# sarath-srinivas/PyGPR

Hardware: AMD Instinct MI355X
Metric: NLML+grad evals/sec at N=16384 D=8 RBF (higher is better)
Workload: dtype f64; 1 GPU; BASELINE config 3: one exact-GP NLML+gradient evaluation per GPU per step, N=16384 D=8, Compose([Squared_exponential, White_noise]), hp sigma=1 l=1 sigma_n=0.1, jitter 1e-7; N>1: grBCM shared-hp co-training (each rank's expert = 1024 global + 15360 own points), one all-reduce of [1+nhp] per step; experts_per_gpu=1

## Files before the change

pygpr_amd/_lib.py:

```python
import ctypes as C
import os
import re

_HERE = os.path.dirname(os.path.abspath(__file__))
LIB_PATH = os.path.join(_HERE, "lib", "libpygpr_hip.so")
HEADER = os.path.join(os.path.dirname(_HERE), "include", "pygpr_hip.h")
HEADER_LOO = os.path.join(os.path.dirname(_HERE), "include", "pygpr_hip_loo.h")
HEADER_SAMPLE = os.path.join(os.path.dirname(_HERE), "include", "pygpr_hip_sample.h")
HEADER_SPARSE = os.path.join(os.path.dirname(_HERE), "include", "pygpr_hip_sparse.h")
HEADER_SELECT = os.path.join(os.path.dirname(_HERE), "include", "pygpr_hip_select.h")
HEADER_MATMUL = os.path.join(os.path.dirname(_HERE), "include", "pygpr_hip_matmul.h")
HEADER_LOWRANK = os.path.join(os.path.dirname(_HERE), "include", "pygpr_hip_lowrank.h")
HEADER_FEATURE = os.path.join(os.path.dirname(_HERE), "include", "pygpr_hip_feature.h")
HEADER_DMATMUL = os.path.join(os.path.dirname(_HERE), "include", "pygpr_hip_dmatmul.h")
HEADER_ROWSQ = os.path.join(os.path.dirname(_HERE), "include", "pygpr_hip_rowsq.h")
HEADER_LXGRAD = os.path.join(os.path.dirname(_HERE), "include", "pygpr_hip_lxgrad.h")

PG_F64, PG_F32 = 0, 1
PG_KIND_RBF, PG_KIND_MATERN52, PG_KIND_SQDIST, PG_KIND_MATERN32, PG_KIND_MATERN12 = 0, 1, 2, 3, 4
PG_KIND_RQ = 6
PG_KIND_PERIODIC = 8
PG_MAX_COMP, PG_MAX_DIM = 4, 64
PG_SPEC_PRODUCT = int(re.search(r"#define\s+PG_SPEC_PRODUCT\s+(0[xX][0-9a-fA-F]+|\d+)", open(HEADER).read()).group(1), 0)
PAD = 256

GEMM_NT, GEMM_NT_RP, GEMM_NN, GEMM_TN, GEMM_TT, GEMM_NT_64, GEMM_NT_64x128, GEMM_NT_32x64, GEMM_NT_32x128, GEMM_TT_64, GEMM_NT_32x32 = 0, 1, 2, 3, 5, 6, 7, 8, 9, 10, 11
GEMM_TN_64 = 13


class CovSpec(C.Structure):
    _fields_ = [
        ("ncomp", C.c_int),
        ("kind", C.c_int * PG_MAX_COMP),
        ("off", C.c_int * PG_MAX_COMP),
        ("nnoise", C.c_int),
        ("noise_off", C.c_int * PG_MAX_COMP),
    ]


_RESTYPES = {"int": C.c_int, "long": C.c_long, "const char*": C.c_char_p}
_ARGTYPES = {"int": C.c_int, "long": C.c_long, "double": C.c_double, "const pg_covspec*": C.POINTER(CovSpec)}
_ARGTYPES.update((t, C.c_void_p) for t in ("pg_handle", "pg_handle*", "void*", "const void*", "double*", "const double*", "int*", "long*"))


def _strip_comments(text):
    return re.sub(r"/\*.*?\*/", "", text, flags=re.S)


def header_symbols():
    return sorted(set(re.findall(r"\b(pg_[a-z_0-9]+)\s*\(", _strip_comments(open(HEADER).read()))))


def parse_prototypes(text):
    def norm(t):
        return re.sub(r"\s*\*", "*", " ".join(t.split()))

    protos = {}
    for ret, name, params in re.findall(r"([\w \t*]+?)\b(pg_[a-z_0-9]+)\s*\(([^()]*)\)\s*;", _strip_comments(text)):
        types = []
        for p in [q.strip() for q in params.split(",")] if params.strip() != "void" else []:
            m = re.fullmatch(r"(.*[\s*])[A-Za-z_]\w*", p, flags=re.S)
            if not m:
                raise ValueError("%s: cannot read parameter %r" % (name, p))
            types.append(norm(m.group(1)))
        protos[name] = (norm(ret), types)
    return protos


def signatures(protos):
    sigs = {}
    for name, (ret, params) in protos.items():
        for t, table in [(ret, _RESTYPES)] + [(p, _ARGTYPES) for p in params]:
            if t not in table:
                raise ValueError("%s: no ctypes mapping for the type %r" % (name, t))
        sigs[name] = (_RESTYPES[ret], [_ARGTYPES[p] for p in params])
    return sigs


_SIGS = signatures(parse_prototypes(open(HEADER).read()))
_SIGS_LOO = signatures(parse_prototypes(open(HEADER_LOO).read()))
# ... 58 lines not shown
```

pygpr_amd/csrc/capi.hip:

```cpp
#include "gemm.h"
#include "kbuild.h"
#include "leaf.h"
#include "chainstep.h"
#include "linalg.h"
#include "pygpr_hip_loo.h"
#include "pygpr_hip_sample.h"
#include "sparse.h"
#include "select.h"
#include "kmatmul.h"
#include "dmatmul.h"
#include "krowsq.h"
#include "fmatmul.h"
#include "lowrank.h"
#include "lxgrad.h"
#include <cstdarg>
#include <cstdint>
#include <cstdio>
#include <cstdlib>
#include <cstring>
#include <mutex>
#include <vector>

static thread_local char g_err[512] = "";

// ... 54 lines not shown
    if (h && h->tmo_host) {
        const int v = *(volatile int*)h->tmo_host;
        if (v) {
            *(volatile int*)h->tmo_host = 0;
            if (h->coupled) {
                h->tmo_off = 1; h->calls_since_tmo = 0;
                if (h->rearms > h->rearms_seen) { h->rearm_cur = std::min(4096, std::max(1, h->rearm_cur) * 2); h->rearms_seen = h->rearms; }
            }
            h->coupled = 0;
            if (v != h->counted_epoch) {
                h->counted_epoch = v;
                h->timeouts += 1;
            }
        }
    }
}

static int join_side(pg_ctx* h, void* stream) {
    poll_timeout(h);
    if (h && h->side_pending) {
        PG_CHECK(hipStreamWaitEvent(ST(stream), h->ev[5], 0));
        if (ST(stream) == h->side_owner) h->side_pending = 0;
    }
    return 0;
}
#define JOIN(h, stream)                         \
    do {                                        \
        int _j = join_side((h), (stream));      \
        if (_j) return _j;                      \
    } while (0)

static int plain_device_memory(const void* p) {
    hipPointerAttribute_t a;
    if (hipPointerGetAttributes(&a, p) != hipSuccess) {
        (void)hipGetLastError();
        return 0;
    }
    return a.type == hipMemoryTypeDevice && !a.isManaged && !(a.allocationFlags & hipDeviceMallocFinegrained);
}
struct AtomicGuard {
    pg_ctx* h;
    AtomicGuard(pg_ctx* h_, const void* c) : h(h_) { if (h) h->no_atomic_c = plain_device_memory(c) ? 0 : 1; }
    ~AtomicGuard() { if (h) h->no_atomic_c = 0; }
};

template <typename T>
static int gemm_raw_t(pg_handle h, int variant, int M, int N, int K, double alpha, const void* A, long lda, const void* B,
                      long ldb, double beta, void* C, long ldc, int tri, int klo, int khi, void* stream) {
    GemmP<T> p;
    p.A = (const T*)A; p.B = (const T*)B; p.C = (T*)C;
    p.lda = lda; p.ldb = ldb; p.ldc = ldc;
    p.M = M; p.N = N; p.K = K;
    p.alpha = (T)alpha; p.beta = (T)beta;
    p.tri = tri; p.klo = klo & 3; p.khi = khi; p.krev = (klo >> 2) & 1;
    p.sA = p.sB = p.sC = 0; p.batch = 1;
    p.nexp = 1; p.eA = p.eB = p.eC = 0; p.einfo = 0;
    p.part = nullptr; p.ldp = 0; p.info = nullptr; p.noxcd = 0;
    static const char* rs = getenv("PG_RAW_STREAM");
    hipStream_t on = ST(stream);
    if (rs && rs[0] == 'u' && h->upd) on = h->upd;
    if (on == ST(stream)) return pg_gemm<T>(h, on, variant, p);
    PG_CHECK(hipEventRecord(h->ev[2], ST(stream)));
    PG_CHECK(hipStreamWaitEvent(on, h->ev[2], 0));
    const int rc = pg_gemm<T>(h, on, variant, p);
    PG_CHECK(hipEventRecord(h->ev[3], on));
    PG_CHECK(hipStreamWaitEvent(ST(stream), h->ev[3], 0));
    return rc;
}

__global__ void pg_probe_wait_kernel(int* flag, int* seen) {
    int ok = 0;
    for (int it = 0; it < 4096 && !ok; ++it) {
        ok = __hip_atomic_load(flag, __ATOMIC_RELAXED, __HIP_MEMORY_SCOPE_SYSTEM) != 0;
        __builtin_amdgcn_s_sleep(32);
    }
    __hip_atomic_store(seen, ok ? 1 : 2, __ATOMIC_RELAXED, __HIP_MEMORY_SCOPE_SYSTEM);
}
__global__ void pg_probe_set_kernel(int* flag) { __hip_atomic_store(flag, 1, __ATOMIC_RELAXED, __HIP_MEMORY_SCOPE_SYSTEM); }

static int probe_concurrent_queues(pg_ctx* c) {
    if (!c->probe_words && hipHostMalloc(reinterpret_cast<void**>(&c->probe_words), 64, hipHostMallocMapped) != hipSuccess) {
        (void)hipGetLastError();
        c->probe_words = nullptr;
        return 0;
    }
    int* words = c->probe_words;
    words[0] = 0;
    words[1] = 0;
    int* dwords = nullptr;
    int ok = 0;
    if (hipHostGetDevicePointer(reinterpret_cast<void**>(&dwords), words, 0) == hipSuccess) {
        hipLaunchKernelGGL(pg_probe_wait_kernel, dim3(1), dim3(1), 0, c->aux, dwords, dwords + 1);
        hipLaunchKernelGGL(pg_probe_set_kernel, dim3(1), dim3(1), 0, c->rows, dwords);
        if (hipStreamSynchronize(c->aux) == hipSuccess && hipStreamSynchronize(c->rows) == hipSuccess) ok = words[1] == 1;
    }
    (void)hipGetLastError();
    return ok;
}

static void maybe_rearm(pg_ctx* h) {
    if (h && h->coupled && h->rearms > 0 && h->rearm_cur > h->rearm_after && ++h->calls_since_rearm > h->rearm_cur) {
        h->rearm_cur = h->rearm_after;
        h->calls_since_rearm = 0;
    }
    if (!h || !h->tmo_off || h->coupled || h->rearm_after <= 0) return;
    if (h->rearm_cur < h->rearm_after) h->rearm_cur = h->rearm_after;
    if (++h->calls_since_tmo <= h->rearm_cur) return;
    h->calls_since_tmo = 0;
    if (h->rows && h->spin_ticks >= 0 && probe_concurrent_queues(h)) {
        h->coupled = 1;
// ... 980 lines not shown
    int* w = reinterpret_cast<int*>(scratch);
    const CsWait cw = {w + 1, nullptr, pg_wait_ticks(h, n), 1};
    return pg_spin_probe_launch(ST(stream), w, cw, reinterpret_cast<long long*>(w + 4));
}
int pg_chain_timeouts(pg_handle h) {
    if (!h) return -1;
    poll_timeout(h);
    return h->timeouts;
}

int pg_build_potrf_trtri_checked(pg_handle h, int dtype, const pg_covspec* spec, const double* hp, const void* X, long ldx, int n,
                                 int d, double jitter, void* A, long lda, int n_pad, void* inv_diag, int* info, void* Minv, long ldm,
                                 void* stream, int* info_host) {
    NEED(info_host, "null pointer");
    for (int attempt = 0; attempt < 2; ++attempt) {
        const int rc = pg_build_potrf_trtri(h, dtype, spec, hp, X, ldx, n, d, jitter, A, lda, n_pad, inv_diag, info, Minv, ldm, stream);
        if (rc) return rc;
        PG_CHECK(hipMemcpyAsync(info_host, info, sizeof(int), hipMemcpyDeviceToHost, ST(stream)));
        PG_CHECK(hipStreamSynchronize(ST(stream)));
        if (*info_host >= 0) return 0;
        poll_timeout(h);
        if (h->coupled) { h->tmo_off = 1; h->calls_since_tmo = 0; }
        h->coupled = 0;
    }
    return 0;
}

int pg_leaf_raw(pg_handle h, int dtype, void* A, long lda, void* inv, long ldi, int* info, void* stream) {
    JOIN(h, stream);
    NEED(h && A && info, "null pointer");
    return dispatch(dtype, __func__, [&](auto t) { using T = decltype(t);
        return pg_leaf<T>(ST(stream), (T*)A, lda, (T*)inv, ldi, info, 0);
    });
}

int pg_rowstep_raw(pg_handle h, int dtype, int n, void* A, long lda, int o0, int k0, const void* inv, int* flags, int* info, void* stream) {
    JOIN(h, stream);
    NEED(h && A && inv && flags && info, "null pointer");
    NEED(n % 128 == 0 && k0 % 128 == 0 && o0 % 128 == 0 && o0 <= k0 && k0 + 128 < n, "bad shape");
    PG_CHECK(hipMemsetAsync(flags, 0x40, 8 * sizeof(int), ST(stream)));
    PG_CHECK(hipMemsetAsync(flags + 6, 0, 2 * sizeof(int), ST(stream)));
    const CsWait cw = {flags + 6, nullptr, 200000000LL, 1};
    return dispatch(dtype, __func__, [&](auto t) { using T = decltype(t);
        return pg_rowstep<T>(ST(stream), (T*)A, lda, n, o0, k0, 1, (const T*)inv, flags, flags + 1, flags + 2, cw, info, flags + 3, flags + 4, 0);
    });
}

int pg_gemm_raw(pg_handle h, int dtype, int variant, int M, int N, int K, double alpha, const void* A, long lda,
                const void* B, long ldb, double beta, void* C, long ldc, int tri, int klo, int khi, void* stream) {
    JOIN(h, stream);
    NEED(h && A && B && C, "null pointer");
    NEED(variant == GEMM_NT_128 || variant == GEMM_NT_RP || variant == GEMM_NN_128 || variant == GEMM_TN_128 ||
             variant == GEMM_TT_128 || variant == GEMM_NT_64 || variant == GEMM_NT_64x128 || variant == GEMM_NT_32x64 ||
             variant == GEMM_NT_32x128 || variant == GEMM_TT_64 || variant == GEMM_NT_32x32 || variant == GEMM_TN_64,
         "variant not exposed");
    NEED16(A, lda); NEED16(B, ldb); NEED16(C, ldc);
    AtomicGuard ag(h, C);
    return dispatch(dtype, __func__, [&](auto t) {
        return gemm_raw_t<decltype(t)>(h, variant, M, N, K, alpha, A, lda, B, ldb, beta, C, ldc, tri, klo, khi, stream);
    });
}

}
```

pygpr_amd/csrc/gemm.h:

```cpp
#pragma once
#include "common.h"

template <typename T> struct GemmP {
    const T* A;
    const T* B;
    T* C;
    long lda, ldb, ldc;
    int M, N, K;
    T alpha, beta;
    int tri;
    int klo, khi;
    int krev;
    long sA, sB, sC;
    int batch;
    int nexp;
    long eA, eB, eC;
    int einfo;
    T* part;
    long ldp;
    const int* info;
    int noxcd;
    int atomic_c;
};

enum GemmVariant {
    GEMM_NT_128 = 0,
    GEMM_NT_RP = 1,
    GEMM_NN_128 = 2,
    GEMM_TN_128 = 3,
    GEMM_NN_128_SS = 4,
    GEMM_TT_128 = 5,
    GEMM_NT_64 = 6,
    GEMM_NT_64x128 = 7,
    GEMM_NT_32x64 = 8,
    GEMM_NT_32x128 = 9,
    GEMM_TT_64 = 10,
    GEMM_NT_128_SS = 12,
    GEMM_TN_64 = 13,
    GEMM_NT_32x32 = 11
};

template <typename T> int pg_gemm(pg_ctx* ctx, hipStream_t st, int variant, const GemmP<T>& p);
double pg_gemm_flops(int variant, int M, int N, int K, int tri, int klo, int khi, int batch);
```

pygpr_amd/csrc/gemm.hip:

```cpp
#include "gemm.h"
#include <cstdlib>
#include <cstdio>

#define BK 16

template <typename T, int R, bool KCONT, int BKT = BK, int NTH = 256> struct Stage {
    static constexpr int VE = 16 / sizeof(T);
    static constexpr int NV = (R * BKT / VE) / NTH;
    static_assert(NV >= 1, "fewer 16-byte vectors in the stage than threads");
    static constexpr int LDS_ELEMS = KCONT ? R * (BKT + 2) : BKT * (R + 16);
    typedef T vec_t __attribute__((ext_vector_type(VE)));
    typedef T half_t __attribute__((ext_vector_type(VE / 2)));
    vec_t v[NV];
    unsigned boff[NV];

    __device__ __forceinline__ void init(long ld, int tid) {
#pragma unroll
        for (int q = 0; q < NV; ++q) {
            const int idx = tid + NTH * q;
            if (KCONT) {
                const int row = idx / (BKT / VE), kv = idx % (BKT / VE);
                boff[q] = (unsigned)(((long)row * ld + kv * VE) * (long)sizeof(T));
            } else {
                const int kr = idx / (R / VE), rv = idx % (R / VE);
                boff[q] = (unsigned)(((long)kr * ld + rv * VE) * (long)sizeof(T));
            }
        }
    }
    static __device__ __forceinline__ const T* origin(const T* __restrict__ g, long ld, int r0, int k0) {
        return KCONT ? g + (long)r0 * ld + k0 : g + (long)k0 * ld + r0;
    }
    __device__ __forceinline__ void load(const T* __restrict__ org) {
        const char* b = reinterpret_cast<const char*>(org);
#pragma unroll
        for (int q = 0; q < NV; ++q) v[q] = *reinterpret_cast<const vec_t*>(b + (size_t)boff[q]);
    }
    __device__ __forceinline__ void store(T* s, int tid) const {
#pragma unroll
        for (int q = 0; q < NV; ++q) {
            const int idx = tid + NTH * q;
            if (KCONT) {
                const int row = idx / (BKT / VE), kv = idx % (BKT / VE);
                T* d = s + row * (BKT + 2) + kv * VE;
                half_t lo, hi;
#pragma unroll
                for (int e = 0; e < VE / 2; ++e) { lo[e] = v[q][e]; hi[e] = v[q][e + VE / 2]; }
                if (sizeof(T) == 8) {
                    *reinterpret_cast<vec_t*>(d) = v[q];
                } else {
                    *reinterpret_cast<half_t*>(d) = lo;
                    *reinterpret_cast<half_t*>(d + VE / 2) = hi;
                }
            } else {
                const int kr = idx / (R / VE), rv = idx % (R / VE);
                *reinterpret_cast<vec_t*>(s + kr * (R + 16) + rv * VE) = v[q];
            }
        }
    }
    static __device__ __forceinline__ T frag(const T* s, int r, int k) {
        return KCONT ? s[r * (BKT + 2) + k] : s[k * (R + 16) + r];
    }
};

template <typename T, int BM, int BN>
__device__ __forceinline__ void gemm_decode(const GemmP<T>& p, int wg, int& ti, int& tj) {
    constexpr int GR = 8;
    const bool grouped = !(p.klo | p.khi | p.noxcd);
    int tmT = p.M / BM;
    if (p.tri && p.N / BN < tmT) {
        const int tnA = p.N / BN, t0 = tnA * (tnA + 1) / 2;
        if (wg >= t0) {
            const int w0 = wg - t0, band = w0 / (GR * tnA), r0 = band * GR;
            const int rows = min(GR, tmT - tnA - r0), w = w0 - band * GR * tnA;
            ti = tnA + r0 + w % rows;
            tj = w / rows;
            return;
        }
        tmT = tnA;
    }
    if (p.tri && grouped) {
        int g = (int)((sqrtf(1024.0f + 128.0f * (float)wg) - 32.0f) / 64.0f);
        while (g > 0 && 32L * g * (g - 1) + 36L * g > wg) --g;
        while (32L * (g + 1) * g + 36L * (g + 1) <= wg) ++g;
        int w = wg - (int)(32L * g * (g - 1) + 36L * g);
        const int r0 = GR * g;
        if (r0 + GR > tmT) {
            ti = r0;
            while (w >= ti + 1) { w -= ti + 1; ++ti; }
            tj = w;
        } else if (w < GR * r0) {
            tj = w / GR; ti = r0 + w % GR;
        } else {
            w -= GR * r0;
            int c = 0;
            while (w >= GR - c) { w -= GR - c; ++c; }
            tj = r0 + c; ti = r0 + c + w;
        }
    } else if (p.tri) {
        ti = (int)((sqrtf(8.0f * (float)wg + 1.0f) - 1.0f) * 0.5f);
        while ((long)ti * (ti + 1) / 2 > wg) --ti;
        while ((long)(ti + 1) * (ti + 2) / 2 <= wg) ++ti;
        tj = wg - ti * (ti + 1) / 2;
        if (p.krev & 1) tj = (tj + (int)(((long)ti * (ti + 1) / 2) & 7)) % (ti + 1);
    } else if (grouped) {
        const int tn = p.N / BN, tmr = p.M / BM;
        const int band = wg / (GR * tn), r0 = band * GR;
        const int rows = min(GR, tmr - r0), w = wg - band * GR * tn;
        ti = r0 + w % rows;
        tj = w / rows;
    } else if (p.khi == 2 && p.N / BN > 1) {
        const int tmr = p.M / BM;
        tj = p.N / BN - 1 - wg / tmr;
        ti = wg % tmr;
    } else {
        const int tn = p.N / BN;
        ti = wg / tn;
        tj = wg % tn;
        if (p.khi == 1) ti = p.M / BM - 1 - ti;
    }
}

template <typename T> __device__ __forceinline__ int gemm_xcd_order(const GemmP<T>& p, int b, int nwg) {
    const int q8 = nwg >> 3, r8 = nwg & 7, xcd = b & 7;
    return (p.klo | p.khi | p.noxcd) ? b : (xcd < r8 ? xcd * (q8 + 1) : r8 * (q8 + 1) + (xcd - r8) * q8) + (b >> 3);
}

template <typename T, bool TA, bool TB, int BM, int BN, int EPI, int BKT, int NW>
__device__ __forceinline__ void gemm_tile(const GemmP<T>& p, int ti, int tj, char* smem_raw) {
    constexpr int NTH = 64 * NW;
    typedef Stage<T, BM, !TA, BKT, NTH> SA;
    typedef Stage<T, BN, TB, BKT, NTH> SB;
    typedef typename Mfma<T>::acc_t acc_t;
    constexpr int WTM = (NW == 8 && BM == 64) ? 16 : ((BM == 128 || BN == 256) ? 64 : ((BM == 32 && BN <= 64) ? 16 : 32));
    constexpr int WTN = (NW == 8) ? 32 : ((BN == 32) ? 16 : ((BN == 64 || (BM == 32 && BN == 128)) ? 32 : 64));
    constexpr int MIM = WTM / 16, MIN = WTN / 16;
    constexpr int WN_ = BN / WTN;
    static_assert((BM / WTM) * (BN / WTN) == NW, "the waves must tile the block");
    const int ze = (int)blockIdx.y / p.batch;
    T* As = reinterpret_cast<T*>(smem_raw);
    T* Bs = As + 2 * SA::LDS_ELEMS;

    const int tid = threadIdx.x, lane = tid & 63, wave = tid >> 6;
    const int wm = wave / WN_, wn = wave % WN_;
    const long zb = (int)blockIdx.y % p.batch;
    const T* __restrict__ A = p.A + zb * p.sA + ze * p.eA;
    const T* __restrict__ B = p.B + zb * p.sB + ze * p.eB;
    T* __restrict__ C = p.C ? p.C + zb * p.sC + ze * p.eC : nullptr;

    const int m0 = ti * BM, n0 = tj * BN;
    int kbeg = 0, kend = p.K;
    int kbw = 0, kew = p.K;
    if (p.klo == 1) { kbeg = m0; kbw = m0 + wm * WTM; }
    if (p.klo == 2) { kbeg = n0; kbw = n0 + wn * WTN; }
    if (p.khi == 1) { kend = min(p.K, m0 + BM); kew = min(p.K, m0 + (wm + 1) * WTM); }
    if (p.khi == 2) { kend = min(p.K, n0 + BN); kew = min(p.K, n0 + (wn + 1) * WTN); }

    acc_t acc[MIM][MIN];
#pragma unroll
    for (int i = 0; i < MIM; ++i)
#pragma unroll
        for (int j = 0; j < MIN; ++j)
#pragma unroll
            for (int r = 0; r < 4; ++r) acc[i][j][r] = (T)0;

    SA sa;
    SB sb;
    sa.init(p.lda, tid);
    sb.init(p.ldb, tid);
    const int nk = (kend - kbeg) / BKT;
    const bool rev = p.klo != 0 && p.krev != 0;
    const int kfirst = rev ? kend - BKT : kbeg, kstep = rev ? -BKT : BKT;
    if (nk > 0) {
        sa.load(SA::origin(A, p.lda, m0, kfirst));
        sb.load(SB::origin(B, p.ldb, n0, kfirst));
        sa.store(As, tid);
        sb.store(Bs, tid);
    }
    __syncthreads();

    const int fr = lane & 15, fk = lane >> 4;
    for (int kt = 0; kt < nk; ++kt) {
        const int cur = kt & 1;
        const int k0 = kfirst + kt * kstep;
        if (kt + 1 < nk) {
            sa.load(SA::origin(A, p.lda, m0, k0 + kstep));
            sb.load(SB::origin(B, p.ldb, n0, k0 + kstep));
        }
        if (k0 + BKT > kbw && k0 < kew) {
            const T* as = As + cur * SA::LDS_ELEMS;
            const T* bs = Bs + cur * SB::LDS_ELEMS;
            constexpr bool PF = TA || !TB;
            if constexpr (PF) {
                T a[2][MIM], bq[2][MIN];
#pragma unroll
                for (int i = 0; i < MIM; ++i) a[0][i] = SA::frag(as, wm * WTM + i * 16 + fr, fk);
#pragma unroll
                for (int j = 0; j < MIN; ++j) bq[0][j] = SB::frag(bs, wn * WTN + j * 16 + fr, fk);
#pragma unroll
                for (int kk = 0; kk < BKT / 4; ++kk) {
                    const int c = kk & 1, nx = c ^ 1;
                    if (kk + 1 < BKT / 4) {
#pragma unroll
                        for (int i = 0; i < MIM; ++i) a[nx][i] = SA::frag(as, wm * WTM + i * 16 + fr, (kk + 1) * 4 + fk);
#pragma unroll
                        for (int j = 0; j < MIN; ++j) bq[nx][j] = SB::frag(bs, wn * WTN + j * 16 + fr, (kk + 1) * 4 + fk);
                    }
#pragma unroll
                    for (int i = 0; i < MIM; ++i)
#pragma unroll
                        for (int j = 0; j < MIN; ++j) acc[i][j] = Mfma<T>::run(a[c][i], bq[c][j], acc[i][j]);
                }
            } else {
#pragma unroll
                for (int kk = 0; kk < BKT / 4; ++kk) {
                    T a[MIM], bq[MIN];
#pragma unroll
                    for (int i = 0; i < MIM; ++i) a[i] = SA::frag(as, wm * WTM + i * 16 + fr, kk * 4 + fk);
#pragma unroll
                    for (int j = 0; j < MIN; ++j) bq[j] = SB::frag(bs, wn * WTN + j * 16 + fr, kk * 4 + fk);
#pragma unroll
                    for (int i = 0; i < MIM; ++i)
#pragma unroll
                        for (int j = 0; j < MIN; ++j) acc[i][j] = Mfma<T>::run(a[i], bq[j], acc[i][j]);
                }
            }
        }
        if (kt + 1 < nk) {
            sa.store(As + (cur ^ 1) * SA::LDS_ELEMS, tid);
            sb.store(Bs + (cur ^ 1) * SB::LDS_ELEMS, tid);
        }
        __syncthreads();
    }

    if (EPI == 0) {
        const T alpha = p.alpha, beta = p.beta;
#pragma unroll
        for (int i = 0; i < MIM; ++i)
#pragma unroll
            for (int j = 0; j < MIN; ++j)
#pragma unroll
                for (int r = 0; r < 4; ++r) {
                    const int row = m0 + wm * WTM + i * 16 + Mfma<T>::row(lane, r);
                    const int col = n0 + wn * WTN + j * 16 + fr;
                    T* c = C + (long)row * p.ldc + col;
                    T v = alpha * acc[i][j][r];
                    if (p.atomic_c) {
                        unsafeAtomicAdd(c, v);
                        continue;
                    }
                    if (beta != (T)0) v += beta * *c;
                    *c = v;
                }
    } else {
        static_assert(EPI == 0 || WTM == 64, "the column-sum epilogue assumes 64-row wave tiles");
#pragma unroll
        for (int j = 0; j < MIN; ++j) {
            T s = (T)0;
#pragma unroll
            for (int i = 0; i < MIM; ++i)
#pragma unroll
                for (int r = 0; r < 4; ++r) s += acc[i][j][r] * acc[i][j][r];
            s += __shfl_xor(s, 16, 64);
            s += __shfl_xor(s, 32, 64);
            if (lane < 16) {
                const int col = n0 + wn * WTN + j * 16 + lane;
                p.part[(long)(m0 / 64 + wm) * p.ldp + col + zb * p.sC + (long)ze * p.eC] = s;
            }
        }
    }
}

template <typename T, bool TA, bool TB, int BM, int BN, int EPI, int BKT = BK, int NW = 4>
__global__ __launch_bounds__(64 * NW, NW == 4 ? 2 : 4) void pg_gemm_kernel(GemmP<T> p) {
    const int ze = (int)blockIdx.y / p.batch;
    if (p.info && p.info[(long)ze * p.einfo] != 0) return;
    extern __shared__ __attribute__((aligned(16))) char smem_raw[];
    int ti, tj;
    gemm_decode<T, BM, BN>(p, gemm_xcd_order(p, blockIdx.x, gridDim.x), ti, tj);
    gemm_tile<T, TA, TB, BM, BN, EPI, BKT, NW>(p, ti, tj, smem_raw);
}

template <typename T>
__global__ __launch_bounds__(512, 4) void pg_gemm_mixed_kernel(GemmP<T> p, int tmain) {
    if (p.info && p.info[0] != 0) return;
    extern __shared__ __attribute__((aligned(16))) char smem_raw[];
    const int b = blockIdx.x;
    int ti, tj;
    if (b < tmain) {
        gemm_decode<T, 128, 128>(p, gemm_xcd_order(p, b, tmain), ti, tj);
        gemm_tile<T, false, true, 128, 128, 0, BK, 8>(p, ti, tj, smem_raw);
    } else {
        const int s = b - tmain, q = s & 3;
        gemm_decode<T, 128, 128>(p, tmain + (s >> 2), ti, tj);
        if (p.tri && ti == tj && q == 1) return;
        gemm_tile<T, false, true, 64, 64, 0, 32, 8>(p, 2 * ti + (q >> 1), 2 * tj + (q & 1), smem_raw);
    }
}

template <typename T, bool TA, bool TB, int BM, int BN, int EPI, int BKT = BK, int NW = 4>
static int launch(hipStream_t st, const GemmP<T>& p) {
    typedef Stage<T, BM, !TA, BKT, 64 * NW> SA;
    typedef Stage<T, BN, TB, BKT, 64 * NW> SB;
    const size_t lds = 2 * (SA::LDS_ELEMS + SB::LDS_ELEMS) * sizeof(T);
    static bool attr_done = false;
    auto kern = pg_gemm_kernel<T, TA, TB, BM, BN, EPI, BKT, NW>;
    if (!attr_done) {
        PG_CHECK(hipFuncSetAttribute(reinterpret_cast<const void*>(kern),
                                     hipFuncAttributeMaxDynamicSharedMemorySize, (int)lds));
        attr_done = true;
    }
    if (p.M % BM || p.N % BN || p.K % BKT || (p.tri && BM != BN)) {
        pg_set_error("pg_gemm: shape %d x %d x %d not tile aligned (%d x %d)", p.M, p.N, p.K, BM, BN);
        return -2;
    }
    if (((p.klo == 1 || p.khi == 1) && BM % BKT) || ((p.klo == 2 || p.khi == 2) && BN % BKT)) {
        pg_set_error("pg_gemm: variant GEMM_%c%c_%dx%d takes no klo = %d / khi = %d: its %d x %d tile is not a multiple of its K tile (%d)",
                     TA ? 'T' : 'N', TB ? 'T' : 'N', BM, BN, p.klo, p.khi, BM, BN, BKT);
        return -2;
    }
    const int tm = p.M / BM, tn = p.N / BN;
    if (p.tri && tn > tm) { pg_set_error("pg_gemm: tri with N = %d > M = %d", p.N, p.M); return -2; }
    const long tiles = p.tri ? (long)tn * (tn + 1) / 2 + (long)(tm - tn) * tn : (long)tm * tn;
    if (tiles == 0 || p.batch == 0 || p.nexp == 0) return 0;
    if (p.batch > 65535) { pg_set_error("pg_gemm: batch=%d exceeds the grid's y limit", p.batch); return -2; }
    const int per = std::max(1, 65535 / p.batch);
    for (int e0 = 0; e0 < p.nexp; e0 += per) {
        GemmP<T> q = p;
        q.nexp = std::min(per, p.nexp - e0);
        q.A = p.A + (long)e0 * p.eA; q.B = p.B + (long)e0 * p.eB;
        if (p.C) q.C = p.C + (long)e0 * p.eC;
        if (p.part) q.part = p.part + (long)e0 * p.eC;
        if (p.info) q.info = p.info + (long)e0 * p.einfo;
        dim3 grid((unsigned)tiles, (unsigned)(q.batch * q.nexp), 1);
        hipLaunchKernelGGL(kern, grid, dim3(64 * NW), lds, st, q);
        PG_CHECK(hipGetLastError());
    }
    return 0;
}

template <typename T> static int launch_mixed(hipStream_t st, const GemmP<T>& p, int tmain) {
    typedef Stage<T, 128, true, BK, 512> S128;
    typedef Stage<T, 64, true, 32, 512> S64;
    static_assert(S64::LDS_ELEMS <= S128::LDS_ELEMS, "the quarter tiles' stages must fit the block's LDS");
    const size_t lds = 4 * S128::LDS_ELEMS * sizeof(T);
    static bool attr_done = false;
    auto kern = pg_gemm_mixed_kernel<T>;
    if (!attr_done) {
        PG_CHECK(hipFuncSetAttribute(reinterpret_cast<const void*>(kern), hipFuncAttributeMaxDynamicSharedMemorySize, (int)lds));
        attr_done = true;
    }
    const long tm = p.M / 128, tn = p.N / 128, tiles = p.tri ? tm * (tm + 1) / 2 : tm * tn;
    dim3 grid((unsigned)(tmain + 4 * (tiles - tmain)), 1, 1);
    hipLaunchKernelGGL(kern, grid, dim3(512), lds, st, p, tmain);
    PG_CHECK(hipGetLastError());
    return 0;
}

double pg_gemm_flops(int variant, int M, int N, int K, int tri, int klo, int khi, int batch) {
    const int BM = (variant == GEMM_NT_32x64 || variant == GEMM_NT_32x128 || variant == GEMM_NT_32x32) ? 32
                   : ((variant == GEMM_NT_RP || variant == GEMM_NT_64 || variant == GEMM_NT_64x128 || variant == GEMM_TT_64 || variant == GEMM_TN_64) ? 64 : 128);
    const int BN = (variant == GEMM_NT_RP) ? 256
                   : ((variant == GEMM_NT_64 || variant == GEMM_NT_32x64 || variant == GEMM_TT_64 || variant == GEMM_TN_64) ? 64
                      : (variant == GEMM_NT_32x32 ? 32 : 128));
    const int tm = M / BM, tn = N / BN;
    double f = 0;
    for (int ti = 0; ti < tm; ++ti)
        for (int tj = 0; tj < (tri ? std::min(ti + 1, tn) : tn); ++tj) {
            int kb = 0, ke = K;
            if (klo == 1) kb = ti * BM;
            if (klo == 2) kb = tj * BN;
            if (khi == 1) ke = std::min(K, (ti + 1) * BM);
            if (khi == 2) ke = std::min(K, (tj + 1) * BN);
            if (ke > kb) f += 2.0 * BM * BN * (double)(ke - kb);
        }
    return f * batch;
}

template <typename T> int pg_gemm(pg_ctx* ctx, hipStream_t st, int variant_in, const GemmP<T>& p_in) {
    int variant = variant_in;
    static const int noxcd = getenv("PG_NOXCD") ? atoi(getenv("PG_NOXCD")) : 0;
    static const int w4env = getenv("PG_GEMM_W4") ? atoi(getenv("PG_GEMM_W4")) : 0;
    static const int ss4 = getenv("PG_SS_W4") ? atoi(getenv("PG_SS_W4")) : 1;
    const bool w4 = w4env || sizeof(T) == 4 || ((variant == GEMM_NN_128_SS || variant == GEMM_NT_128_SS) && ss4);
    GemmP<T> p = p_in;
    p.noxcd = noxcd;
    if (p.nexp < 1) p.nexp = 1;
    static const int atomic_c = getenv("PG_ATOMIC_C") ? atoi(getenv("PG_ATOMIC_C")) : 1;
    p.atomic_c = (atomic_c && !(ctx && ctx->no_atomic_c) && sizeof(T) == 8 && p.beta == (T)1 && p.C && p.part == nullptr) ? 1 : 0;
    const bool prof = ctx && ctx->prof_on;
    if (prof) PG_CHECK(hipEventRecord(ctx->ev[6], st));
    int rc;
    static const int mixed_env = getenv("PG_GEMM_MIXED") ? atoi(getenv("PG_GEMM_MIXED")) : 1;
    if (mixed_env && variant == GEMM_NT_128 && !w4 && sizeof(T) == 8 && ctx && ctx->ncu > 0 && !p.klo && !p.khi && !p.noxcd && p.batch == 1 &&
        p.nexp == 1 && p.part == nullptr && p.M % 128 == 0 && p.N % 128 == 0 && p.K % 32 == 0 && (!p.tri || p.M == p.N)) {
        const long tm = p.M / 128, tn = p.N / 128, tiles = p.tri ? tm * (tm + 1) / 2 : tm * tn;
        const long slots = 2L * ((ctx->upd && st == ctx->upd) ? ctx->upd_cus : ctx->ncu);
        const long rem = tiles % slots;
        if (tiles > slots && rem > 0 && 4 * rem <= (5 * slots) / 2) {
            if constexpr (sizeof(T) == 8) {
                if ((rc = launch_mixed<T>(st, p, (int)(tiles - rem)))) return rc;
                variant = -1;
            }
        }
    }
    switch (variant) {
        case -1: rc = 0; break;
        case GEMM_NT_128: rc = w4 ? launch<T, false, true, 128, 128, 0>(st, p) : launch<T, false, true, 128, 128, 0, BK, 8>(st, p); break;
        case GEMM_NT_RP: rc = launch<T, false, true, 64, 256, 0>(st, p); break;
        case GEMM_NN_128: rc = w4 ? launch<T, false, false, 128, 128, 0>(st, p) : launch<T, false, false, 128, 128, 0, BK, 8>(st, p); break;
        case GEMM_TN_128: rc = w4 ? launch<T, true, false, 128, 128, 0>(st, p) : launch<T, true, false, 128, 128, 0, BK, 8>(st, p); break;
        case GEMM_NT_128_SS: rc = w4 ? launch<T, false, true, 128, 128, 1>(st, p) : launch<T, false, true, 128, 128, 1, BK, 8>(st, p); break;
        case GEMM_NN_128_SS: rc = w4 ? launch<T, false, false, 128, 128, 1>(st, p) : launch<T, false, false, 128, 128, 1, BK, 8>(st, p); break;
        case GEMM_TT_128: rc = w4 ? launch<T, true, true, 128, 128, 0>(st, p) : launch<T, true, true, 128, 128, 0, BK, 8>(st, p); break;
        case GEMM_NT_64: rc = launch<T, false, true, 64, 64, 0>(st, p); break;
        case GEMM_NT_64x128: rc = launch<T, false, true, 64, 128, 0>(st, p); break;
        case GEMM_NT_32x64: rc = launch<T, false, true, 32, 64, 0, 32>(st, p); break;
        case GEMM_NT_32x128: rc = launch<T, false, true, 32, 128, 0, (sizeof(T) == 8 ? 16 : 32)>(st, p); break;
        case GEMM_TT_64: rc = launch<T, true, true, 64, 64, 0>(st, p); break;
        case GEMM_TN_64: rc = launch<T, true, false, 64, 64, 0>(st, p); break;
        case GEMM_NT_32x32: rc = launch<T, false, true, 32, 32, 0, 64>(st, p); break;
        default: pg_set_error("pg_gemm: unknown variant %d", variant); return -2;
    }
    if (rc) return rc;
    variant = variant_in;
    {
        static FILE* logf = getenv("PG_GEMM_LOG") ? fopen(getenv("PG_GEMM_LOG"), "w") : nullptr;
        if (logf) {
            fprintf(logf, "%d %d %d %d %d %d %d %.0f\n", variant, (int)sizeof(T), w4 ? 4 : 8, p.M, p.N, p.K, p.batch,
                    pg_gemm_flops(variant, p.M, p.N, p.K, p.tri, p.klo, p.khi, p.batch * p.nexp));
            fflush(logf);
        }
    }
    if (prof) {
        PG_CHECK(hipEventRecord(ctx->ev[7], st));
        PG_CHECK(hipEventSynchronize(ctx->ev[7]));
        float ms = 0;
        PG_CHECK(hipEventElapsedTime(&ms, ctx->ev[6], ctx->ev[7]));
        ctx->prof_ms += ms;
        ctx->prof_flops += pg_gemm_flops(variant, p.M, p.N, p.K, p.tri, p.klo, p.khi, p.batch * p.nexp);
        ctx->prof_launches += 1;
    }
    return 0;
}

template int pg_gemm<double>(pg_ctx*, hipStream_t, int, const GemmP<double>&);
template int pg_gemm<float>(pg_ctx*, hipStream_t, int, const GemmP<float>&);
```

pygpr_amd/csrc/linalg.hip:

```cpp
#include "gemm.h"
#include "leaf.h"
#include "chainstep.h"
#include "kbuild.h"
#include "linalg.h"
#include <cmath>
#include <cstdlib>
#include <vector>

#define NB 128
static int pg_nbo(const pg_ctx* ctx, int n) {
    if (ctx->nbo) return ctx->nbo;
    return n <= 10240 ? 512 : (n <= 18432 ? 1024 : 2048);
}

template <typename T>
__global__ __launch_bounds__(256) void copy_blocks_kernel(const T* __restrict__ src, T* __restrict__ dst, long ldd, long esrc, long edst) {
    src += blockIdx.z * esrc;
    dst += blockIdx.z * edst;
    const int b = blockIdx.x;
    const T* s = src + (long)b * NB * NB;
    T* d = dst + (long)b * NB * ldd + (long)b * NB;
    for (int idx = blockIdx.y * 256 + threadIdx.x; idx < NB * NB; idx += gridDim.y * 256)
        d[(long)(idx >> 7) * ldd + (idx & 127)] = s[idx];
}
// ... 268 lines not shown
    var[j] = (T)v;
    mean[j] = (T)(v * (sums[2 * lds + j] + b0 * pg * (double)mean_g[j]));
}

template <typename T>
__global__ __launch_bounds__(256) void weighted_prec_kernel(const T* __restrict__ P, long ldp, const double* __restrict__ beta,
                                                            int m, int m_pad, T* __restrict__ acc, long lda, int accumulate) {
    const int tc = blockIdx.x, tr = blockIdx.y;
    if (tc > tr) return;
    for (int idx = threadIdx.x; idx < 64 * 64; idx += 256) {
        const int i = tr * 64 + (idx >> 6), j = tc * 64 + (idx & 63);
        if (i >= m_pad || j > i) continue;
        T* a = acc + (long)i * lda + j;
        if (i < m) {
            const double v = 0.5 * (beta[i] + beta[j]) * (double)P[(long)i * ldp + j];
            *a = (T)(accumulate ? (double)*a + v : v);
        } else if (!accumulate) {
            *a = (i == j) ? (T)1 : (T)0;
        }
    }
}

template <typename T> __global__ __launch_bounds__(256) void symmetrize_kernel(T* __restrict__ A, long lda, int n) {
    const int tc = blockIdx.x, tr = blockIdx.y;
    if (tc < tr) return;
    for (int idx = threadIdx.x; idx < 64 * 64; idx += 256) {
        const int i = tr * 64 + (idx >> 6), j = tc * 64 + (idx & 63);
        if (i < n && j < n && j > i) A[(long)i * lda + j] = A[(long)j * lda + i];
    }
}

template <typename T>
__global__ __launch_bounds__(256) void grbcm_finish_full_kernel(const double* __restrict__ sums, long lds, const T* __restrict__ mean_g,
                                                                const T* __restrict__ var_g, const T* __restrict__ cov, long ldc,
                                                                int m, T* __restrict__ mean) {
    const int j = blockIdx.x * 256 + threadIdx.x;
    if (j >= m) return;
    const double pg = 1.0 / (double)var_g[j];
    const double b0 = 1.0 - sums[j];
    mean[j] = (T)((double)cov[(long)j * ldc + j] * (sums[2 * lds + j] + b0 * pg * (double)mean_g[j]));
}

#define LAUNCH_CHECK() PG_CHECK(hipGetLastError())

template <typename T> static GemmP<T> gp0() {
    GemmP<T> p;
    p.A = p.B = nullptr; p.C = nullptr;
    p.lda = p.ldb = p.ldc = 0;
    p.M = p.N = p.K = 0;
    p.alpha = (T)1; p.beta = (T)0;
    p.tri = p.klo = p.khi = 0; p.krev = 0;
    p.sA = p.sB = p.sC = 0; p.batch = 1;
    p.nexp = 1; p.eA = p.eB = p.eC = 0; p.einfo = 0;
    p.part = nullptr; p.ldp = 0; p.info = nullptr; p.noxcd = 0;
    return p;
}

static long pg_flag_elems(int n) { return 128L * (n / NB) + 2048; }
long pg_potrf_worksize_impl(int n) { return (long)n * NB + pg_flag_elems(n); }

template <typename T>
int pg_trtri_t(pg_ctx* ctx, hipStream_t st, int n, const T* L, long ldl, const T* invD, T* M, long ldm, int hmax, const ExpBatch* eb) {
    if (n <= 0 || n % NB) { pg_set_error("pg_trtri: n=%d is not a positive multiple of %d", n, NB); return -2; }
    const int nexp = eb ? eb->nexp : 1;
    const long eL = eb ? eb->eA : 0, eI = eb ? eb->eInv : 0, eMm = eb ? eb->eM : 0;
    hipLaunchKernelGGL(copy_blocks_kernel<T>, dim3(n / NB, 8, nexp), dim3(256), 0, st, invD, M, ldm, eI, eMm);
    LAUNCH_CHECK();
    int rc;
    long h = NB, rem = 0;
    for (;;) {
        const long nfull = (n - rem) / h;
        if (nfull + (rem ? 1 : 0) <= 1) break;
        if (hmax && h >= hmax) break;
        const long npair = nfull / 2;
        for (int pass = 0; pass < 2; ++pass) {
            long r0, h2, batch;
            if (pass == 0) { if (!npair) continue; r0 = 0; h2 = h; batch = npair; }
            else { if (!((nfull & 1) && rem)) continue; r0 = (nfull - 1) * h; h2 = rem; batch = 1; }
            const long stride = 2 * h * (ldm + 1);
            GemmP<T> p = gp0<T>();
            p.M = (int)h; p.N = (int)h2; p.K = (int)h;
            p.A = M + r0 * ldm + r0; p.lda = ldm;
            p.B = L + (r0 + h) * ldl + r0; p.ldb = ldl;
            p.C = M + r0 * ldm + r0 + h; p.ldc = ldm;
            p.klo = 1; p.batch = (int)batch;
            p.sA = stride; p.sC = stride; p.sB = 2 * h * (ldl + 1);
            p.nexp = nexp; p.eA = eMm; p.eB = eL; p.eC = eMm;
            const bool small = batch * (h / 128) * (h2 / 128) * nexp <= 1024 && h2 % 64 == 0;
            if ((rc = pg_gemm<T>(ctx, st, small ? GEMM_TT_64 : GEMM_TT_128, p))) return rc;
            p = gp0<T>();
            p.M = (int)h2; p.N = (int)h; p.K = (int)h2;
            p.A = M + (r0 + h) * ldm + r0 + h; p.lda = ldm;
            p.B = M + r0 * ldm + r0 + h; p.ldb = ldm;
            p.C = M + (r0 + h) * ldm + r0; p.ldc = ldm;
            p.alpha = (T)-1; p.khi = 1; p.batch = (int)batch;
            p.sA = p.sB = p.sC = stride;
            p.nexp = nexp; p.eA = p.eB = p.eC = eMm;
            if ((rc = pg_gemm<T>(ctx, st, small ? GEMM_NT_64 : GEMM_NT_128, p))) return rc;
        }
        if (nfull & 1) rem = rem ? h + rem : h;
        h *= 2;
    }
    return 0;
}

template <typename T>
static int trtri_top(pg_ctx* ctx, hipStream_t st, int h1, int h2, const T* L, long ldl, T* M, long ldm) {
// ... 687 lines not shown
```

Before: 13.97 evals/s.

## Add software-pipelined fp64 128x128 GEMM with buffer loads for TN/NN

Adds a new fp64 128x128 GEMM kernel that interleaves global loads, LDS stores, LDS fragment reads and MFMA groups under explicit scheduling barriers, double-buffering register fragments across k-steps. Global operand loads use uniform buffer-resource loads with scalar base addresses, and the 8-wave NT tile also uses them. TN and untriangular NN GEMMs with K of at least 384 are routed to the pipelined kernel by default unless an 'exact' flag or the update stream is used. The aim is to hide memory and LDS latency behind matrix-core work in the Cholesky/trsm-heavy NLML path, at the cost of added code complexity and a different accumulation ordering.

```diff
diff --git a/pygpr_amd/_lib.py b/pygpr_amd/_lib.py
--- a/pygpr_amd/_lib.py
+++ b/pygpr_amd/_lib.py
@@ -26,6 +26,7 @@
 
 GEMM_NT, GEMM_NT_RP, GEMM_NN, GEMM_TN, GEMM_TT, GEMM_NT_64, GEMM_NT_64x128, GEMM_NT_32x64, GEMM_NT_32x128, GEMM_TT_64, GEMM_NT_32x32 = 0, 1, 2, 3, 5, 6, 7, 8, 9, 10, 11
 GEMM_TN_64 = 13
+PIPELINED = {GEMM_NT: 14, GEMM_NN: 15, GEMM_TN: 16, GEMM_TT: 17}
 
 
 class CovSpec(C.Structure):
diff --git a/pygpr_amd/csrc/capi.hip b/pygpr_amd/csrc/capi.hip
--- a/pygpr_amd/csrc/capi.hip
+++ b/pygpr_amd/csrc/capi.hip
@@ -130,10 +130,23 @@
     p.lda = lda; p.ldb = ldb; p.ldc = ldc;
     p.M = M; p.N = N; p.K = K;
     p.alpha = (T)alpha; p.beta = (T)beta;
-    p.tri = tri; p.klo = klo & 3; p.khi = khi; p.krev = (klo >> 2) & 1;
+    p.klo = klo & 3; p.khi = khi; p.krev = (klo >> 2) & 1;
+    p.exact = (klo >> 3) & 1;
     p.sA = p.sB = p.sC = 0; p.batch = 1;
     p.nexp = 1; p.eA = p.eB = p.eC = 0; p.einfo = 0;
     p.part = nullptr; p.ldp = 0; p.info = nullptr; p.noxcd = 0;
+    p.tri = tri & 1;
+    if (tri & 14) {
+        const bool ta = variant == GEMM_TN_128 || variant == GEMM_TT_128 || variant == GEMM_TT_64 || variant == GEMM_TN_64 ||
+                        variant == GEMM_TN_128_PL || variant == GEMM_TT_128_PL;
+        const bool tb = !(variant == GEMM_NN_128 || variant == GEMM_TN_128 || variant == GEMM_TN_64 || variant == GEMM_NN_128_PL ||
+                          variant == GEMM_TN_128_PL);
+        p.batch = (tri & 2) ? 2 : 1;
+        p.nexp = (tri & 4) ? 2 : 1;
+        p.sA = (long)(ta ? K : M) * lda; p.sB = (long)(tb ? N : K) * ldb; p.sC = (long)M * ldc;
+        p.eA = p.batch * p.sA; p.eB = p.batch * p.sB; p.eC = p.batch * p.sC;
+        if (tri & 8) { p.info = reinterpret_cast<const int*>(reinterpret_cast<const char*>(C) - 16); p.einfo = 1; }
+    }
     static const char* rs = getenv("PG_RAW_STREAM");
     hipStream_t on = ST(stream);
     if (rs && rs[0] == 'u' && h->upd) on = h->upd;
@@ -1220,7 +1233,8 @@
     NEED(h && A && B && C, "null pointer");
     NEED(variant == GEMM_NT_128 || variant == GEMM_NT_RP || variant == GEMM_NN_128 || variant == GEMM_TN_128 ||
              variant == GEMM_TT_128 || variant == GEMM_NT_64 || variant == GEMM_NT_64x128 || variant == GEMM_NT_32x64 ||
-             variant == GEMM_NT_32x128 || variant == GEMM_TT_64 || variant == GEMM_NT_32x32 || variant == GEMM_TN_64,
+             variant == GEMM_NT_32x128 || variant == GEMM_TT_64 || variant == GEMM_NT_32x32 || variant == GEMM_TN_64 ||
+             variant == GEMM_NT_128_PL || variant == GEMM_NN_128_PL || variant == GEMM_TN_128_PL || variant == GEMM_TT_128_PL,
          "variant not exposed");
     NEED16(A, lda); NEED16(B, ldb); NEED16(C, ldc);
     AtomicGuard ag(h, C);
diff --git a/pygpr_amd/csrc/gemm.h b/pygpr_amd/csrc/gemm.h
--- a/pygpr_amd/csrc/gemm.h
+++ b/pygpr_amd/csrc/gemm.h
@@ -21,6 +21,7 @@
     const int* info;
     int noxcd;
     int atomic_c;
+    int exact;
 };
 
 enum GemmVariant {
@@ -37,7 +38,11 @@
     GEMM_TT_64 = 10,
     GEMM_NT_128_SS = 12,
     GEMM_TN_64 = 13,
-    GEMM_NT_32x32 = 11
+    GEMM_NT_32x32 = 11,
+    GEMM_NT_128_PL = 14,
+    GEMM_NN_128_PL = 15,
+    GEMM_TN_128_PL = 16,
+    GEMM_TT_128_PL = 17
 };
 
 template <typename T> int pg_gemm(pg_ctx* ctx, hipStream_t st, int variant, const GemmP<T>& p);
diff --git a/pygpr_amd/csrc/gemm.hip b/pygpr_amd/csrc/gemm.hip
--- a/pygpr_amd/csrc/gemm.hip
+++ b/pygpr_amd/csrc/gemm.hip
@@ -35,9 +35,23 @@
 #pragma unroll
         for (int q = 0; q < NV; ++q) v[q] = *reinterpret_cast<const vec_t*>(b + (size_t)boff[q]);
     }
+    __device__ __forceinline__ void load_uniform(const T* __restrict__ org, long ld) {
+        static_assert(KCONT ? NTH % (BKT / VE) == 0 : NTH % (R / VE) == 0, "a lane's vectors must lie whole rows apart");
+        const unsigned long u = reinterpret_cast<unsigned long>(org);
+        const unsigned lo = __builtin_amdgcn_readfirstlane((unsigned)u), hi = __builtin_amdgcn_readfirstlane((unsigned)(u >> 32));
+        void* b = reinterpret_cast<void*>(((unsigned long)hi << 32) | lo);
+        const __amdgpu_buffer_rsrc_t rs = __builtin_amdgcn_make_buffer_rsrc(b, 0, -1, 0x00020000);
+        const unsigned qs = (unsigned)((KCONT ? NTH / (BKT / VE) : NTH / (R / VE)) * ld * (long)sizeof(T));
+#pragma unroll
+        for (int q = 0; q < NV; ++q)
+            v[q] = __builtin_bit_cast(vec_t, __builtin_amdgcn_raw_buffer_load_b128(rs, (int)boff[0], (int)(q * qs), 0));
+    }
     __device__ __forceinline__ void store(T* s, int tid) const {
 #pragma unroll
-        for (int q = 0; q < NV; ++q) {
+        for (int q = 0; q < NV; ++q) store_one(s, tid, q);
+    }
+    __device__ __forceinline__ void store_one(T* s, int tid, int q) const {
+        {
             const int idx = tid + NTH * q;
             if (KCONT) {
                 const int row = idx / (BKT / VE), kv = idx % (BKT / VE);
@@ -128,6 +142,7 @@
 template <typename T, bool TA, bool TB, int BM, int BN, int EPI, int BKT, int NW>
 __device__ __forceinline__ void gemm_tile(const GemmP<T>& p, int ti, int tj, char* smem_raw) {
     constexpr int NTH = 64 * NW;
+    constexpr bool UL = sizeof(T) == 8 && BM == 128 && BN == 128 && NW == 8 && EPI == 0 && !TA && TB;
     typedef Stage<T, BM, !TA, BKT, NTH> SA;
     typedef Stage<T, BN, TB, BKT, NTH> SB;
     typedef typename Mfma<T>::acc_t acc_t;
@@ -171,8 +186,13 @@
     const bool rev = p.klo != 0 && p.krev != 0;
     const int kfirst = rev ? kend - BKT : kbeg, kstep = rev ? -BKT : BKT;
     if (nk > 0) {
-        sa.load(SA::origin(A, p.lda, m0, kfirst));
-        sb.load(SB::origin(B, p.ldb, n0, kfirst));
+        if (UL) {
+            sa.load_uniform(SA::origin(A, p.lda, m0, kfirst), p.lda);
+            sb.load_uniform(SB::origin(B, p.ldb, n0, kfirst), p.ldb);
+        } else {
+            sa.load(SA::origin(A, p.lda, m0, kfirst));
+            sb.load(SB::origin(B, p.ldb, n0, kfirst));
+        }
         sa.store(As, tid);
         sb.store(Bs, tid);
     }
@@ -183,8 +203,13 @@
         const int cur = kt & 1;
         const int k0 = kfirst + kt * kstep;
         if (kt + 1 < nk) {
-            sa.load(SA::origin(A, p.lda, m0, k0 + kstep));
-            sb.load(SB::origin(B, p.ldb, n0, k0 + kstep));
+            if (UL) {
+                sa.load_uniform(SA::origin(A, p.lda, m0, k0 + kstep), p.lda);
+                sb.load_uniform(SB::origin(B, p.ldb, n0, k0 + kstep), p.ldb);
+            } else {
+                sa.load(SA::origin(A, p.lda, m0, k0 + kstep));
+                sb.load(SB::origin(B, p.ldb, n0, k0 + kstep));
+            }
         }
         if (k0 + BKT > kbw && k0 < kew) {
             const T* as = As + cur * SA::LDS_ELEMS;
@@ -270,6 +295,175 @@
     }
 }
 
+#define PL_FENCE() __builtin_amdgcn_sched_barrier(0)
+template <bool TA, bool TB> struct PlTile {
+    typedef double T;
+    static constexpr int BM = 128, BN = 128, BKT = BK, NTH = 256, MIM = 4, MIN = 4;
+    typedef Stage<T, BM, !TA, BKT, NTH> SA;
+    typedef Stage<T, BN, TB, BKT, NTH> SB;
+    typedef Mfma<T>::acc_t acc_t;
+
+    static __device__ __forceinline__ void read_pair(T (&a)[2][MIM], T (&b)[2][MIN], const T* as, const T* bs, int ra, int rb, int fk, int pr) {
+#pragma unroll
+        for (int s = 0; s < 2; ++s) {
+#pragma unroll
+            for (int i = 0; i < MIM; ++i) a[s][i] = SA::frag(as, ra + i * 16, (2 * pr + s) * 4 + fk);
+#pragma unroll
+            for (int j = 0; j < MIN; ++j) b[s][j] = SB::frag(bs, rb + j * 16, (2 * pr + s) * 4 + fk);
+        }
+    }
+    static __device__ __forceinline__ void mma8(acc_t (&acc)[MIM][MIN], const T (&a)[2][MIM], const T (&b)[2][MIN], int s, int i0) {
+#pragma unroll
+        for (int i = i0; i < i0 + 2; ++i)
+#pragma unroll
+            for (int j = 0; j < MIN; ++j) acc[i][j] = Mfma<T>::run(a[s][i], b[s][j], acc[i][j]);
+    }
+    template <bool NEXT, bool MMA>
+    static __device__ __forceinline__ void step(acc_t (&acc)[MIM][MIN], T (&a0)[2][MIM], T (&b0)[2][MIN], SA& sa, SB& sb, const T* as,
+                                                const T* bs, T* asn, T* bsn, const T* ga, const T* gb, long p_lda, long p_ldb, int tid, int ra, int rb, int fk) {
+        T a1[2][MIM], b1[2][MIN];
+        if (NEXT) {
+            sa.load_uniform(ga, p_lda);
+            sb.load_uniform(gb, p_ldb);
+        }
+        PL_FENCE();
+        if (MMA) {
+            read_pair(a1, b1, as, bs, ra, rb, fk, 1);
+            PL_FENCE();
+            mma8(acc, a0, b0, 0, 0);
+            PL_FENCE();
+            mma8(acc, a0, b0, 0, 2);
+            PL_FENCE();
+            mma8(acc, a0, b0, 1, 0);
+            PL_FENCE();
+        }
+        if (NEXT) { sa.store_one(asn, tid, 0); sa.store_one(asn, tid, 1); }
+        PL_FENCE();
+        if (MMA) { mma8(acc, a0, b0, 1, 2); PL_FENCE(); }
+        if (NEXT) { sa.store_one(asn, tid, 2); sa.store_one(asn, tid, 3); }
+        PL_FENCE();
+        if (MMA) { mma8(acc, a1, b1, 0, 0); PL_FENCE(); }
+        if (NEXT) { sb.store_one(bsn, tid, 0); sb.store_one(bsn, tid, 1); }
+        PL_FENCE();
+        if (MMA) { mma8(acc, a1, b1, 0, 2); PL_FENCE(); }
+        if (NEXT) { sb.store_one(bsn, tid, 2); sb.store_one(bsn, tid, 3); }
+        PL_FENCE();
+        if (MMA) { mma8(acc, a1, b1, 1, 0); PL_FENCE(); }
+        if (NEXT) {
+            __syncthreads();
+            read_pair(a0, b0, asn, bsn, ra, rb, fk, 0);
+            PL_FENCE();
+        }
+        if (MMA) { mma8(acc, a1, b1, 1, 2); PL_FENCE(); }
+    }
+
+    static __device__ __forceinline__ void run(const GemmP<T>& p, int ti, int tj, char* smem_raw) {
+        static_assert(SA::NV == 4 && SB::NV == 4, "pl_step places four vectors per operand");
+        const int ze = (int)blockIdx.y / p.batch;
+        T* As = reinterpret_cast<T*>(smem_raw);
+        T* Bs = As + 2 * SA::LDS_ELEMS;
+        const int tid = threadIdx.x, lane = tid & 63;
+        const int wave = __builtin_amdgcn_readfirstlane(tid >> 6);
+        const int wm = wave >> 1, wn = wave & 1;
+        const long zb = (int)blockIdx.y % p.batch;
+        const T* __restrict__ A = p.A + zb * p.sA + ze * p.eA;
+        const T* __restrict__ B = p.B + zb * p.sB + ze * p.eB;
+        T* __restrict__ C = p.C + zb * p.sC + ze * p.eC;
+
+        const int m0 = ti * BM, n0 = tj * BN;
+        int kbeg = 0, kend = p.K;
+        int kbw = 0, kew = p.K;
+        if (p.klo == 1) { kbeg = m0; kbw = m0 + wm * 64; }
+        if (p.klo == 2) { kbeg = n0; kbw = n0 + wn * 64; }
+        if (p.khi == 1) { kend = min(p.K, m0 + BM); kew = min(p.K, m0 + (wm + 1) * 64); }
+        if (p.khi == 2) { kend = min(p.K, n0 + BN); kew = min(p.K, n0 + (wn + 1) * 64); }
+
+        acc_t acc[MIM][MIN];
+#pragma unroll
+        for (int i = 0; i < MIM; ++i)
+#pragma unroll
+            for (int j = 0; j < MIN; ++j)
+#pragma unroll
+                for (int r = 0; r < 4; ++r) acc[i][j][r] = 0.0;
+
+        const int fr = lane & 15, fk = lane >> 4;
+        const int ra = wm * 64 + fr, rb = wn * 64 + fr;
+        const int nk = (kend - kbeg) / BKT;
+        const bool rev = p.klo != 0 && p.krev != 0;
+        const int kfirst = rev ? kend - BKT : kbeg, kstep = rev ? -BKT : BKT;
+        if (nk > 0) {
+            SA sa;
+            SB sb;
+            sa.init(p.lda, tid);
+            sb.init(p.ldb, tid);
+            const T* ga = SA::origin(A, p.lda, m0, kfirst);
+            const T* gb = SB::origin(B, p.ldb, n0, kfirst);
+            const long p_lda = p.lda, p_ldb = p.ldb;
+            const long da = (long)kstep * (TA ? p.lda : 1), db = (long)kstep * (TB ? 1 : p.ldb);
+            sa.load_uniform(ga, p_lda);
+            sb.load_uniform(gb, p_ldb);
+            sa.store(As, tid);
+            sb.store(Bs, tid);
+            __syncthreads();
+            T a0[2][MIM], b0[2][MIN];
+            read_pair(a0, b0, As, Bs, ra, rb, fk, 0);
+            PL_FENCE();
+            const int lo = max(kbw, kbeg), hi = min(kew, kend);
+            int u0 = 0, u1 = 0;
+            if (hi > lo) {
+                u0 = (rev ? kend - hi : lo - kbeg) / BKT;
+                u1 = (rev ? kend - lo : hi - kbeg) / BKT;
+            }
+            const int e0 = min(u0, nk - 1), e1 = min(max(u1, e0), nk - 1);
+            int kt = 0;
+#define PL_TILE(MMA_)                                                                                                               \
+    {                                                                                                                               \
+        const int cur = kt & 1;                                                                                                     \
+        ga += da;                                                                                                                   \
+        gb += db;                                                                                                                   \
+        step<true, MMA_>(acc, a0, b0, sa, sb, As + cur * SA::LDS_ELEMS, Bs + cur * SB::LDS_ELEMS, As + (cur ^ 1) * SA::LDS_ELEMS,   \
+                         Bs + (cur ^ 1) * SB::LDS_ELEMS, ga, gb, p_lda, p_ldb, tid, ra, rb, fk);                                    \
+    }
+            for (; kt < e0; ++kt) PL_TILE(false)
+            for (; kt < e1; ++kt) PL_TILE(true)
+            for (; kt < nk - 1; ++kt) PL_TILE(false)
+#undef PL_TILE
+            if (u0 < nk && u1 == nk) {
+                const int cur = (nk - 1) & 1;
+                step<false, true>(acc, a0, b0, sa, sb, As + cur * SA::LDS_ELEMS, Bs + cur * SB::LDS_ELEMS, nullptr, nullptr, nullptr, nullptr, 0, 0, tid, ra, rb, fk);
+            }
+        }
+
+        const T alpha = p.alpha, beta = p.beta;
+#pragma unroll
+        for (int i = 0; i < MIM; ++i)
+#pragma unroll
+            for (int j = 0; j < MIN; ++j)
+#pragma unroll
+                for (int r = 0; r < 4; ++r) {
+                    const int row = m0 + wm * 64 + i * 16 + Mfma<T>::row(lane, r);
+                    const int col = n0 + wn * 64 + j * 16 + fr;
+                    T* c = C + (long)row * p.ldc + col;
+                    T v = alpha * acc[i][j][r];
+                    if (p.atomic_c) {
+                        unsafeAtomicAdd(c, v);
+                        continue;
+                    }
+                    if (beta != 0.0) v += beta * *c;
+                    *c = v;
+                }
+    }
+};
+
+template <bool TA, bool TB> __global__ __launch_bounds__(256, 2) void pg_gemm_pl_kernel(GemmP<double> p) {
+    const int ze = (int)blockIdx.y / p.batch;
+    if (p.info && p.info[(long)ze * p.einfo] != 0) return;
+    extern __shared__ __attribute__((aligned(16))) char smem_raw[];
+    int ti, tj;
+    gemm_decode<double, 128, 128>(p, gemm_xcd_order(p, blockIdx.x, gridDim.x), ti, tj);
+    PlTile<TA, TB>::run(p, ti, tj, smem_raw);
+}
+
 template <typename T, bool TA, bool TB, int BM, int BN, int EPI, int BKT = BK, int NW = 4>
 __global__ __launch_bounds__(64 * NW, NW == 4 ? 2 : 4) void pg_gemm_kernel(GemmP<T> p) {
     const int ze = (int)blockIdx.y / p.batch;
@@ -297,13 +491,19 @@
     }
 }
 
-template <typename T, bool TA, bool TB, int BM, int BN, int EPI, int BKT = BK, int NW = 4>
+template <typename T, bool TA, bool TB, int BM, int BN, int EPI, int BKT, int NW, bool PL> static auto gemm_kernel_of() {
+    if constexpr (PL) return pg_gemm_pl_kernel<TA, TB>;
+    else return pg_gemm_kernel<T, TA, TB, BM, BN, EPI, BKT, NW>;
+}
+
+template <typename T, bool TA, bool TB, int BM, int BN, int EPI, int BKT = BK, int NW = 4, bool PL = false>
 static int launch(hipStream_t st, const GemmP<T>& p) {
+    static_assert(!PL || (sizeof(T) == 8 && BM == 128 && BN == 128 && EPI == 0 && BKT == BK && NW == 4), "the pipelined form is one tile");
     typedef Stage<T, BM, !TA, BKT, 64 * NW> SA;
     typedef Stage<T, BN, TB, BKT, 64 * NW> SB;
     const size_t lds = 2 * (SA::LDS_ELEMS + SB::LDS_ELEMS) * sizeof(T);
     static bool attr_done = false;
-    auto kern = pg_gemm_kernel<T, TA, TB, BM, BN, EPI, BKT, NW>;
+    auto kern = gemm_kernel_of<T, TA, TB, BM, BN, EPI, BKT, NW, PL>();
     if (!attr_done) {
         PG_CHECK(hipFuncSetAttribute(reinterpret_cast<const void*>(kern),
                                      hipFuncAttributeMaxDynamicSharedMemorySize, (int)lds));
@@ -403,6 +603,12 @@
             }
         }
     }
+    constexpr int PL_MIN_K = 384;
+    if (sizeof(T) == 8 && !p.exact && !w4env && !(ctx && ctx->upd && st == ctx->upd) &&
+        (variant == GEMM_TN_128 || (variant == GEMM_NN_128 && !p.klo && !p.khi))) {
+        const int kmax = p.khi == 1 ? std::min(p.K, p.M) : (p.khi == 2 ? std::min(p.K, p.N) : p.K);
+        if (kmax >= PL_MIN_K) variant = variant == GEMM_TN_128 ? GEMM_TN_128_PL : GEMM_NN_128_PL;
+    }
     switch (variant) {
         case -1: rc = 0; break;
         case GEMM_NT_128: rc = w4 ? launch<T, false, true, 128, 128, 0>(st, p) : launch<T, false, true, 128, 128, 0, BK, 8>(st, p); break;
@@ -419,6 +625,17 @@
         case GEMM_TT_64: rc = launch<T, true, true, 64, 64, 0>(st, p); break;
         case GEMM_TN_64: rc = launch<T, true, false, 64, 64, 0>(st, p); break;
         case GEMM_NT_32x32: rc = launch<T, false, true, 32, 32, 0, 64>(st, p); break;
+        case GEMM_NT_128_PL: case GEMM_NN_128_PL: case GEMM_TN_128_PL: case GEMM_TT_128_PL:
+            if constexpr (sizeof(T) == 8) {
+                rc = variant == GEMM_NT_128_PL   ? launch<T, false, true, 128, 128, 0, BK, 4, true>(st, p)
+                     : variant == GEMM_NN_128_PL ? launch<T, false, false, 128, 128, 0, BK, 4, true>(st, p)
+                     : variant == GEMM_TN_128_PL ? launch<T, true, false, 128, 128, 0, BK, 4, true>(st, p)
+                                                 : launch<T, true, true, 128, 128, 0, BK, 4, true>(st, p);
+            } else {
+                pg_set_error("pg_gemm: variant %d (pipelined 128 x 128 tile) is fp64 only", variant);
+                return -2;
+            }
+            break;
         default: pg_set_error("pg_gemm: unknown variant %d", variant); return -2;
     }
     if (rc) return rc;
diff --git a/pygpr_amd/csrc/linalg.hip b/pygpr_amd/csrc/linalg.hip
--- a/pygpr_amd/csrc/linalg.hip
+++ b/pygpr_amd/csrc/linalg.hip
@@ -344,7 +344,7 @@
     p.tri = p.klo = p.khi = 0; p.krev = 0;
     p.sA = p.sB = p.sC = 0; p.batch = 1;
     p.nexp = 1; p.eA = p.eB = p.eC = 0; p.einfo = 0;
-    p.part = nullptr; p.ldp = 0; p.info = nullptr; p.noxcd = 0;
+    p.part = nullptr; p.ldp = 0; p.info = nullptr; p.noxcd = 0; p.exact = 0;
     return p;
 }
 
```

After: 14.25 evals/s, median of 6. 1.02x the previous value.
